# julienperriercornet/turbosqueeze

Hardware: AMD Instinct MI355X
Metric: encode+decode GB/s on enwik9-shaped input (round trip of uncompressed bytes) (higher is better)
Workload: dtype u8

## Files before the change

turbosqueeze_amd/csrc/tsq_enc_stage.cuh:

```cuda
#pragma once
#ifndef TSQ_LATE_FIX
#define TSQ_LATE_FIX 1
#endif
#ifndef TSQ_LM
#define TSQ_LM 4
#endif
#ifndef TSQ_LF
#define TSQ_LF 3
#endif
#ifndef TSQ_LM_LEAN
#define TSQ_LM_LEAN 4
#endif
#ifndef TSQ_LF_LEAN
#define TSQ_LF_LEAN 3
#endif

#include "tsq_common.cuh"
#include "tsq_experiment.h"
#include "tsq_enc_util.cuh"
#include "tsq_enc_builder.cuh"

namespace tsq {

typedef uint32_t u32x4_t __attribute__((ext_vector_type(4)));
// ... 222 lines not shown
    }
    return twin_in;
}

template <bool WINDOW>
__device__ __forceinline__ void stage_in(uint32_t n, lds_u8_t* lds, uint32_t lane)
{
    using StageCfg = StageCfgT<WINDOW>;
    volatile lds_u32_t* recs = (volatile lds_u32_t*)(lds + StageCfg::off_rec);
    lds_u32_t* ctl = (lds_u32_t*)(lds + StageCfg::off_ctl);
    const uint32_t n_tiles = (n >> 6) + 3u;
    uint32_t hashed_seen = 0, slot = 0;
    const uint64_t below_me = below(lane);
#ifdef TSQ_STATS
    unsigned long long st_[32] = {0};
#endif
    TSQ_BEGIN();
    for (uint32_t t = 0; t < n_tiles; ++t, slot = slot + 1u == StageCfg::R ? 0u : slot + 1u) {
        if (!stage_wait_seen(ctl, kCtlHashed, t + 1u, hashed_seen, 0)) break;
        volatile lds_u32_t* arr = recs + slot * StageCfg::REC_WORDS + StageCfg::ARR + lane * 4u;
        const u32x4_t gb = lds_ld4(arr + kGB);
        const uint32_t h = gb.y, own = gb.x;
        const uint64_t twin_in = in_tile_twins(h, own, below_me);
        lds_st2(arr + kGB + 2u, (uint32_t)twin_in, (uint32_t)(twin_in >> 32));
        TSQ_DELAY(10);
        stage_publish(ctl, kCtlIn, t + 1u, lane);
    }
#ifdef TSQ_STATS
    if (blockIdx.x == 0 && lane == 0) { g_enc_stats[34] = st_[22]; g_enc_stats[57] = st_[0]; g_enc_stats[58] = TSQ_TOTAL(); }
#endif
}

template <bool WINDOW>
__device__ __forceinline__ void stage_twins(uint32_t n, lds_u8_t* lds, uint32_t lane)
{
    using StageCfg = StageCfgT<WINDOW>;
    constexpr uint32_t LM = StageCfg::LM;
    volatile lds_u32_t* recs = (volatile lds_u32_t*)(lds + StageCfg::off_rec);
    lds_u32_t* ctl = (lds_u32_t*)(lds + StageCfg::off_ctl);
    const uint32_t n_tiles = (n >> 6) + 3u;
    uint32_t h_m1 = 0xFFFFFFFFu, h_m2 = 0xFFFFFFFFu, h_m3 = 0xFFFFFFFFu, h_m4 = 0xFFFFFFFFu;
    uint32_t hashed_seen = 0, slot = 0;
#ifdef TSQ_STATS
    unsigned long long st_[32] = {0};
#endif
    TSQ_BEGIN();
    for (uint32_t t = 0; t < n_tiles; ++t, slot = slot + 1u == StageCfg::R ? 0u : slot + 1u) {
        if (!stage_wait_seen(ctl, StageCfg::SPLIT_IN ? kCtlIn : kCtlHashed, t + 1u, hashed_seen, 0)) break;
        volatile lds_u32_t* rec = recs + slot * StageCfg::REC_WORDS;
        volatile lds_u32_t* arr = rec + StageCfg::ARR + lane * 4u;
        const u32x4_t gb = lds_ld4(arr + kGB);
        const uint32_t h = gb.y, own = gb.x;
        const uint32_t before = own & 0xFFu;
        if (!StageCfg::SPLIT_IN) {
            const uint64_t twin_in = in_tile_twins(h, own, below(lane));
            lds_st2(arr + kGB + 2u, (uint32_t)twin_in, (uint32_t)(twin_in >> 32));
        }
        uint64_t twin_p1 = 0, twin_p2 = 0, twin_p3 = 0, twin_p4 = 0;
        bool unsure = false;
        const uint32_t d0 = (t - (before >> 6)) & 3u;
        const uint32_t d = d0 ? d0 : 4u;
        const bool live = d <= t && d <= LM;
        if (__ballot(live) != 0ull) {
            const uint32_t q = before & 63u;
            const uint32_t dd = live ? d : 1u;
            const uint32_t qslot = slot >= dd ? slot - dd : slot + StageCfg::R - dd;
            volatile lds_u32_t* qa = recs + qslot * StageCfg::REC_WORDS + StageCfg::ARR + q * 4u;
            const u32x4_t qb = lds_ld4(qa + kGB);
            const u32x4_t qc = lds_ld4(qa + kGC);
            const uint32_t hq = qb.y;
            const uint64_t q_in = (uint64_t)qb.z | ((uint64_t)qb.w << 32);
            const uint64_t q_p1 = (uint64_t)qc.x | ((uint64_t)qc.y << 32);
            const uint64_t q_p2 = (uint64_t)qc.z | ((uint64_t)qc.w << 32);
            uint64_t q_p3 = 0;
            if (LM == 4u) { const u32x2_t qd = lds_ld2(qa + kGD); q_p3 = (uint64_t)qd.x | ((uint64_t)qd.y << 32); }
            const bool owns = live && StageCfg::fold(hq) == StageCfg::fold(h);
            const bool same = owns && hq == h;
            unsure = owns && hq != h;
            const uint64_t chain = q_in | (1ull << q);
            if (same) {
                twin_p1 = d == 1u ? chain : 0ull;
                twin_p2 = d == 2u ? chain : d == 1u ? q_p1 : 0ull;
                twin_p3 = d == 3u ? chain : d == 2u ? q_p1 : d == 1u ? q_p2 : 0ull;
                if (LM == 4u) twin_p4 = d == 4u ? chain : d == 3u ? q_p1 : d == 2u ? q_p2 : q_p3;
            }
        }
        {
            uint64_t maybe = __ballot(unsure);
            TSQ_CNT(20, __builtin_popcountll(maybe));
            while (maybe) {
                TSQ_CNT(21, 1);
                const uint32_t hl = rdlane(h, lsb64(maybe));
                const uint64_t g1 = __ballot(h_m1 == hl), g2 = __ballot(h_m2 == hl), g3 = __ballot(h_m3 == hl);
                const uint64_t g4 = LM == 4u ? __ballot(h_m4 == hl) : 0ull;
                const uint64_t grp_cur = __ballot(h == hl);
                if (h == hl) { twin_p1 = g1; twin_p2 = g2; twin_p3 = g3; twin_p4 = g4; }
                maybe &= ~grp_cur;
            }
        }
        lds_st4(arr + kGC, (uint32_t)twin_p1, (uint32_t)(twin_p1 >> 32), (uint32_t)twin_p2, (uint32_t)(twin_p2 >> 32));
        lds_st4(arr + kGD, (uint32_t)twin_p3, (uint32_t)(twin_p3 >> 32), (uint32_t)twin_p4, (uint32_t)(twin_p4 >> 32));
        TSQ_TRACE(2, t);
        TSQ_DELAY(1);
        stage_publish(ctl, 2, t + 1u, lane);
        h_m4 = h_m3; h_m3 = h_m2; h_m2 = h_m1; h_m1 = h;
    }
#ifdef TSQ_STATS
    if (blockIdx.x == 0 && lane == 0) { g_enc_stats[48] = st_[0]; g_enc_stats[49] = TSQ_TOTAL(); g_enc_stats[32] = st_[20]; g_enc_stats[33] = st_[21]; }
#endif
}

template <bool EXT, bool WINDOW>
__device__ __forceinline__ void stage_near(uint32_t n, lds_u8_t* lds, uint32_t lane)
{
    using StageCfg = StageCfgT<WINDOW>;
    volatile lds_u32_t* recs = (volatile lds_u32_t*)(lds + StageCfg::off_rec);
    lds_u32_t* ctl = (lds_u32_t*)(lds + StageCfg::off_ctl);
    const uint32_t n_tiles = (n >> 6) + 3u;
    uint32_t scanned_seen = 0, slot = 0;
#ifdef TSQ_STATS
    unsigned long long st_[32] = {0};
#endif
    TSQ_BEGIN();
    for (uint32_t t = 0; t < n_tiles; ++t, slot = slot + 1u == StageCfg::R ? 0u : slot + 1u) {
        if (!stage_wait_seen(ctl, 2, t + 1u, scanned_seen, 0)) break;
        volatile lds_u32_t* rec = recs + slot * StageCfg::REC_WORDS;
        volatile lds_u32_t* arr = rec + StageCfg::ARR + lane * 4u;
        const u32x2_t gi = lds_ld2(arr + kGB + 2u);
        const u32x4_t gc = lds_ld4(arr + kGC);
        u32x2_t gd; gd.x = 0; gd.y = 0;
        if (StageCfg::LM == 4u) gd = lds_ld2(arr + kGD);
        const uint32_t tin_lo = gi.x, tin_hi = gi.y, tp1_lo = gc.x, tp1_hi = gc.y, tp2_lo = gc.z, tp2_hi = gc.w, tp3_lo = gd.x, tp3_hi = gd.y;
        const bool in0 = (tin_lo | tin_hi) != 0u, in1 = (tp1_lo | tp1_hi) != 0u, in2 = (tp2_lo | tp2_hi) != 0u, in3 = (tp3_lo | tp3_hi) != 0u;
        uint32_t word = 0;
        if (__ballot(in0 || in1 || in2 || in3) != 0ull) {
            const uint32_t m_lo = in0 ? tin_lo : in1 ? tp1_lo : in2 ? tp2_lo : tp3_lo, m_hi = in0 ? tin_hi : in1 ? tp1_hi : in2 ? tp2_hi : tp3_hi;
            const uint32_t q = m_hi ? 63u - (uint32_t)__builtin_clz(m_hi) : 31u - (uint32_t)__builtin_clz(m_lo | 1u);
            const uint32_t back = in0 ? 0u : in1 ? 1u : in2 ? 2u : 3u;
            const uint32_t qslot = slot >= back ? slot - back : slot + StageCfg::R - back;
            const u32x4_t a = *(volatile lds_u32x4_t*)(rec + StageCfg::W16 + lane * 4u);
            const u32x4_t b = *(volatile lds_u32x4_t*)(recs + qslot * StageCfg::REC_WORDS + StageCfg::W16 + q * 4u);
            const uint32_t k = prefix16(make_uint4(a.x, a.y, a.z, a.w), make_uint4(b.x, b.y, b.z, b.w));
            if ((in0 || in1 || in2 || in3) && !(EXT && k >= 16u)) word = 0x8000u | (back << 12) | (q << 6) | k;
        }
        arr[kGB] = word;
        TSQ_DELAY(2);
        stage_publish(ctl, kCtlNear, t + 1u, lane);
    }
#ifdef TSQ_STATS
    if (blockIdx.x == 0 && lane == 0) { g_enc_stats[55] = st_[0]; g_enc_stats[56] = TSQ_TOTAL(); }
#endif
}

template <bool EXT, bool WINDOW>
__device__ __forceinline__ void stage_match(const uint8_t* src, uint64_t avail, uint32_t n, uint16_t* table, lds_u8_t* lds, uint32_t lane, uint32_t parity)
{
    using StageCfg = StageCfgT<WINDOW>;
    volatile lds_u32_t* recs = (volatile lds_u32_t*)(lds + StageCfg::off_rec);
    lds_u32_t* ctl = (lds_u32_t*)(lds + StageCfg::off_ctl);
    constexpr uint32_t kDMin = EXT ? 128u : 64u;
    constexpr uint32_t LM = StageCfg::LM;
    const uint32_t tail_from = n >= 5u ? n - 5u : 0u;
    const uint32_t n_tiles = (n >> 6) + 3u;
    uint32_t wbase = parity << 6;
    uint32_t scanned_seen = 0, committed_seen = 0;
#ifdef TSQ_STATS
    unsigned long long st_[32] = {0};
#endif
    TSQ_BEGIN();
    for (uint32_t t = parity; t < n_tiles; t += 2u) {
        MREG_BEGIN(10);
        if (!stage_wait_seen(ctl, 2, t + 1u, scanned_seen, 2)) break;
        TSQ_TRACE(3, t);
        volatile lds_u32_t* rec = recs + (t % StageCfg::R) * StageCfg::REC_WORDS;
        volatile lds_u32_t* arr = rec + StageCfg::ARR + lane * 4u;
        const u32x4_t gb = lds_ld4(arr + kGB);
        const u32x4_t wv = *(volatile lds_u32x4_t*)(rec + StageCfg::W16 + lane * 4u);
        const u32x4_t gc = lds_ld4(arr + kGC);
        const u32x4_t gd = lds_ld4(arr + kGD);
        const uint32_t h = gb.y;
        const uint4 w16 = make_uint4(wv.x, wv.y, wv.z, wv.w);
        const uint64_t twin_in = (uint64_t)gb.z | ((uint64_t)gb.w << 32);
        const uint64_t twin_p1 = (uint64_t)gc.x | ((uint64_t)gc.y << 32);
        const uint32_t tpw_any = LM == 4u ? (gc.z | gc.w | gd.x | gd.y) : (gc.z | gc.w);
        const uint32_t tpm_lo = LM == 4u ? gd.z : gd.x, tpm_hi = LM == 4u ? gd.w : gd.y;
        MREG_END(10);
        MREG_BEGIN(12);
#ifndef TSQ_X_NOCOMMITWAIT
        if (t >= LM + 1u && !stage_wait_seen(ctl, kCtlCommitted, t - LM, committed_seen, 3)) break;
#endif
        TSQ_TRACE(10, t);
#ifdef TSQ_X_FAKE_TABLE
        const uint32_t tv_old = table[h & 0xFFu];
#else
        const uint32_t tv_old = table[h];
#endif
        MREG_END(12);
        MREG_BEGIN(11);
        uint32_t tv = tv_old;
#ifdef TSQ_X_NOPATCH
        if (false) {
#else
        if (t >= LM) {
#endif
            volatile lds_u32_t* vis = recs + ((t - LM) % StageCfg::R) * StageCfg::REC_WORDS + 2u;
            uint32_t vis_lo, vis_hi;
            {
                const uint32_t seen_v = ((volatile lds_u32_t*)ctl)[5];
                uint32_t a = vis[0], b = vis[1];
                asm volatile("" ::: "memory");
                if (uniform(seen_v) < t - LM + 1u) {
                    if (!stage_wait_tight(ctl, 5, t - LM + 1u, 3)) break;
                    a = vis[0]; b = vis[1];
                }
                vis_lo = uniform(a); vis_hi = uniform(b);
            }
            TSQ_TRACE(4, t);
            const uint32_t hit_lo = tpm_lo & vis_lo, hit_hi = tpm_hi & vis_hi;
            const uint32_t q = hit_hi ? 63u - (uint32_t)__builtin_clz(hit_hi) : 31u - (uint32_t)__builtin_clz(hit_lo | 1u);
            if ((hit_lo | hit_hi) != 0u) tv = (((t - LM) << 6) + q) & 0xFFFFu;
        }
        MREG_END(11);
        const uint32_t p = (t << 6) + lane;
        const uint32_t cand0 = candidate_of(tv, p);
        MREG_BEGIN(13);
        uint4 cb;
        if (WINDOW) {
            int32_t wi = (int32_t)(wbase + lane) - (int32_t)(p - cand0);
            wi += wi < 0 ? (int32_t)StageCfg::WIN : 0;
            volatile lds_u32_t* wp = (volatile lds_u32_t*)(lds + StageCfg::off_win + ((uint32_t)wi & ~3u));
            const uint32_t d0 = wp[0], d1 = wp[1], d2 = wp[2], d3 = wp[3], d4 = wp[4];
            const uint32_t sh = (uint32_t)wi & 3u;
            cb = make_uint4(__builtin_amdgcn_alignbyte(d1, d0, sh), __builtin_amdgcn_alignbyte(d2, d1, sh),
                            __builtin_amdgcn_alignbyte(d3, d2, sh), __builtin_amdgcn_alignbyte(d4, d3, sh));
            if (cand0 + 19u > ((t + 1u) << 6) || p - cand0 > 65536u) cb = ld128z(src, cand0, avail);
        }
#ifdef TSQ_X_FAKE_CAND
        else cb = ld128z(src, p, avail);
#else
        else cb = ld128z(src, cand0, avail);
#endif
        uint32_t k0 = prefix16(w16, cb);
        MREG_END(13);
        MREG_BEGIN(14);
        if (EXT) {
            uint32_t more = 16;
            if (__ballot(k0 == more) != 0ull) {
                const uint32_t scanned = uniform(__hip_atomic_load(&ctl[2], __ATOMIC_RELAXED, __HIP_MEMORY_SCOPE_WORKGROUP));
                const bool in_window = WINDOW && scanned >= t + 2u;
                auto win16 = [&](int32_t wi) -> uint4 {
                    wi += wi < 0 ? (int32_t)StageCfg::WIN : 0;
                    wi -= wi >= (int32_t)StageCfg::WIN ? (int32_t)StageCfg::WIN : 0;
                    volatile lds_u32_t* wp = (volatile lds_u32_t*)(lds + StageCfg::off_win + ((uint32_t)wi & ~3u));
                    const uint32_t d0 = wp[0], d1 = wp[1], d2 = wp[2], d3 = wp[3], d4 = wp[4];
                    const uint32_t sh = (uint32_t)wi & 3u;
                    return make_uint4(__builtin_amdgcn_alignbyte(d1, d0, sh), __builtin_amdgcn_alignbyte(d2, d1, sh),
                                      __builtin_amdgcn_alignbyte(d3, d2, sh), __builtin_amdgcn_alignbyte(d4, d3, sh));
                };
                while (__ballot(k0 == more) != 0ull && more < 64u) {
                    TSQ_CNT(20, in_window ? 1 : 0); TSQ_CNT(21, 1);
                    if (k0 == more) {
                        if (in_window && p - cand0 <= 65536u)
                            k0 += prefix16(win16((int32_t)(wbase + lane + more)), win16((int32_t)(wbase + lane + more) - (int32_t)(p - cand0)));
                        else
                            k0 += prefix16(ld128z(src, (uint64_t)p + more, avail), ld128z(src, (uint64_t)cand0 + more, avail));
                    }
                    more += 16;
                }
            }
        }
        const uint32_t dist = p - cand0;
        const bool eq4 = k0 >= 4u;
        const bool far_enough = dist >= kDMin && dist <= 0xFFFEu;
        const bool tail = p >= tail_from;
        bool neart = false;
        if (__ballot((twin_in | twin_p1) != 0ull) != 0ull) {
            const uint64_t near_in = twin_in & ~below(lane >= 3u ? lane - 3u : 0u);
            const uint64_t near_prev = lane < 3u ? twin_p1 & ~below(61u + lane) : 0ull;
            neart = (near_in | near_prev) != 0ull && !tail;
        }
        const bool certain = eq4 && far_enough && !tail && !neart;
        const uint32_t nib = length_nibble(k0 < 4u ? 4u : k0);
        const uint32_t span_nat = certain ? nibble_span(nib) : 1u;
        const bool hard_l = (eq4 && !far_enough && dist >= 4u && !neart) || tail;
        const bool twin_l = (twin_in | twin_p1) != 0ull || tpw_any != 0u;
        lds_st2(arr + kGA, span_nat | (hard_l ? 0x100u : 0u) | (twin_l ? 0x200u : 0u) | (certain ? 0x400u : 0u) | (neart ? 0x800u : 0u) | (k0 << 16),
                cand0 | (nib << 24));
#ifdef TSQ_STATS
        if (t >= 3u) { st_[24] += (uint32_t)((uint32_t)__builtin_amdgcn_s_memtime() - uniform(ctl[40u + ((t - 3u) & 7u)])); st_[25] += 1; }
#endif
        TSQ_TRACE(5, t);
        TSQ_DELAY(3);
        stage_publish(ctl, parity ? kCtlMatchedOdd : 3u, t + 1u, lane);
        MREG_END(14);
        wbase = wbase + 128u >= StageCfg::WIN ? wbase + 128u - StageCfg::WIN : wbase + 128u;
    }
#ifdef TSQ_STATS
    if (blockIdx.x == 0 && lane == 0 && parity == 0u) { g_enc_stats[2] = st_[2]; g_enc_stats[3] = st_[3]; g_enc_stats[4] = TSQ_TOTAL(); g_enc_stats[13] = st_[13]; g_enc_stats[14] = st_[14]; g_enc_stats[35] = st_[20]; g_enc_stats[36] = st_[21]; g_enc_stats[51] = st_[24]; g_enc_stats[52] = st_[25]; }
#endif
}

template <bool WINDOW>
__device__ __forceinline__ void stage_commit(uint32_t n, uint16_t* table, lds_u8_t* lds, uint32_t lane)
{
    using StageCfg = StageCfgT<WINDOW>;
    volatile lds_u32_t* recs = (volatile lds_u32_t*)(lds + StageCfg::off_rec);
    lds_u32_t* ctl = (lds_u32_t*)(lds + StageCfg::off_ctl);
    const uint32_t n_tiles = (n >> 6) + 3u;
#ifdef TSQ_STATS
    unsigned long long st_[32] = {0};
#endif
    TSQ_BEGIN();
    for (uint32_t t = 0; t < n_tiles; ++t) {
        volatile lds_u32_t* rec = recs + (t % StageCfg::R) * StageCfg::REC_WORDS;
        volatile lds_u32_t* arr = rec + StageCfg::ARR + lane * 4u;
        if (!stage_wait(ctl, 5, t + 1u, 3)) break;
        TSQ_TRACE(12, t);
        const u32x4_t gb = lds_ld4(arr + kGB);
        const uint32_t h = gb.y, tin_lo = gb.z, tin_hi = gb.w;
        const uint64_t tw = __ballot((tin_lo | tin_hi) != 0u);
        lds_u32_t* visw = (lds_u32_t*)(rec + 2u);
        const uint64_t vis = (uint64_t)uniform(__hip_atomic_load(&visw[0], __ATOMIC_RELAXED, __HIP_MEMORY_SCOPE_WORKGROUP)) |
                             ((uint64_t)uniform(__hip_atomic_load(&visw[1], __ATOMIC_RELAXED, __HIP_MEMORY_SCOPE_WORKGROUP)) << 32);
        const uint32_t p = (t << 6) + lane;
#ifdef TSQ_X_FAKE_TABLE
#define TSQ_TBL(hh) ((hh) & 0xFFu)
#else
#define TSQ_TBL(hh) (hh)
#endif
        if (((vis & ~tw) >> lane) & 1ull) table[TSQ_TBL(h)] = (uint16_t)p;
        uint64_t late = vis & tw;
        while (late) {
            const uint32_t top = msb64(late);
            if (lane == top) table[TSQ_TBL(h)] = (uint16_t)p;
            late &= ~((uint64_t)rdlane(tin_lo, top) | ((uint64_t)rdlane(tin_hi, top) << 32) | (1ull << top));
        }
        asm volatile("s_waitcnt vmcnt(0)" ::: "memory");
        TSQ_TRACE(6, t);
        TSQ_DELAY(4);
        stage_publish(ctl, kCtlCommitted, t + 1u, lane);
    }
#ifdef TSQ_STATS
    if (blockIdx.x == 0 && lane == 0) { g_enc_stats[45] = st_[3] + st_[4]; g_enc_stats[46] = TSQ_TOTAL(); }
#endif
}

template <bool EXT, bool WINDOW>
__device__ __forceinline__ void stage_orbit(uint32_t n, lds_u8_t* lds, uint32_t lane, uint32_t parity)
{
    using StageCfg = StageCfgT<WINDOW>;
    volatile lds_u32_t* recs = (volatile lds_u32_t*)(lds + StageCfg::off_rec);
    lds_u32_t* ctl = (lds_u32_t*)(lds + StageCfg::off_ctl);
    constexpr uint32_t kDMin = EXT ? 128u : 64u;
    constexpr uint32_t LM = StageCfg::LM, LF = StageCfg::LF;
    const uint32_t tail_from = n >= 5u ? n - 5u : 0u;
    const uint32_t n_tiles = (n >> 6) + 3u;
#ifdef TSQ_STATS
    unsigned long long st_[32] = {0};
#endif
    TSQ_BEGIN();
    uint32_t scanned_seen = 0, parsed_seen = 0, near_seen = 0;
    for (uint32_t t = parity; t < n_tiles; t += 2u) {
        volatile lds_u32_t* rec = recs + (t % StageCfg::R) * StageCfg::REC_WORDS;
        volatile lds_u32_t* arr = rec + StageCfg::ARR + lane * 4u;
        uint32_t fix_sw = 0, fix_lw = 0;
        bool fix = false, clear_far = false;
        if (TSQ_LATE_FIX && t >= LF) {
            if (!stage_wait_seen(ctl, 2, t + 1u, scanned_seen, 6)) break;
            const u32x4_t gc = lds_ld4(arr + kGC);
            const u32x2_t gi = lds_ld2(arr + kGB + 2u);
            u32x2_t gd; gd.x = 0; gd.y = 0;
            if (LM == 4u) gd = lds_ld2(arr + kGD);
            const uint32_t tp_lo[4] = {0u, gc.x, gc.z, gd.x}, tp_hi[4] = {0u, gc.y, gc.w, gd.y};
            uint32_t nearer = gi.x | gi.y, far = 0;
#pragma unroll
            for (uint32_t k = 1; k < LM; ++k) { if (k < LF) nearer |= tp_lo[k] | tp_hi[k]; else far |= tp_lo[k] | tp_hi[k]; }
            const uint32_t p = (t << 6) + lane;
            const bool only_far = far != 0u && nearer == 0u && p < tail_from;
            if (__ballot(only_far) != 0ull) {
                if (!stage_wait_seen(ctl, 5, t - LF + 1u, parsed_seen, 5)) break;
                uint32_t hit_lo = 0, hit_hi = 0, back = 0;
#pragma unroll
                for (uint32_t k = LM - 1u; k >= LF; --k) {
                    lds_u32_t* vis = (lds_u32_t*)(recs + ((t - k) % StageCfg::R) * StageCfg::REC_WORDS + 2u);
                    const uint32_t v_lo = uniform(__hip_atomic_load(&vis[0], __ATOMIC_RELAXED, __HIP_MEMORY_SCOPE_WORKGROUP));
                    const uint32_t v_hi = uniform(__hip_atomic_load(&vis[1], __ATOMIC_RELAXED, __HIP_MEMORY_SCOPE_WORKGROUP));
                    const uint32_t h_lo = tp_lo[k] & v_lo, h_hi = tp_hi[k] & v_hi;
                    if ((h_lo | h_hi) != 0u) { hit_lo = h_lo; hit_hi = h_hi; back = k; }
                }
                clear_far = only_far;
                if (only_far && (hit_lo | hit_hi) != 0u) {
                    const uint32_t q = hit_hi ? 63u - (uint32_t)__builtin_clz(hit_hi) : 31u - (uint32_t)__builtin_clz(hit_lo);
                    const uint32_t cand = (t << 6) - (back << 6) + q;
                    const uint32_t tq = t - back;
                    const u32x4_t a = *(volatile lds_u32x4_t*)(rec + StageCfg::W16 + lane * 4u);
                    const u32x4_t b = *(volatile lds_u32x4_t*)(recs + (tq % StageCfg::R) * StageCfg::REC_WORDS + StageCfg::W16 + q * 4u);
                    const uint32_t k = prefix16(make_uint4(a.x, a.y, a.z, a.w), make_uint4(b.x, b.y, b.z, b.w));
                    if (p - cand >= kDMin && !(EXT && k >= 16u)) {
                        const bool eq4 = k >= 4u;
                        const uint32_t nib = length_nibble(eq4 ? k : 4u);
                        fix_sw = (eq4 ? nibble_span(nib) | 0x400u : 1u) | (k << 16);
                        fix_lw = cand | (nib << 24);
                        fix = true;
                    } else clear_far = false;
                }
            }
        }
        uint32_t sw, lw;
        {
            const uint32_t seen_v = ((volatile lds_u32_t*)ctl)[parity ? kCtlMatchedOdd : 3u];
            u32x2_t ga = lds_ld2(arr + kGA);
            asm volatile("" ::: "memory");
            if (uniform(seen_v) < t + 1u) {
                if (!stage_wait_tight(ctl, parity ? kCtlMatchedOdd : 3u, t + 1u, 6)) break;
                ga = lds_ld2(arr + kGA);
            }
            sw = ga.x; lw = ga.y;
        }
        TSQ_TRACE(11, t);
        if (clear_far) fix_sw |= 0x1000u;
        if (fix) { sw = fix_sw; lw = fix_lw; }
        else if (clear_far) sw |= 0x1000u;
        const uint32_t self = lane | ((sw & 0x100u) ? 0x80u : 0u);
        const uint32_t c = lane + (sw & 0xFFu);
        const uint32_t there = (uint32_t)__builtin_amdgcn_ds_bpermute((int)((c & 63u) << 2), (int)self);
        uint32_t nx = c >= 64u ? (c | 0x80u) : there;
        uint64_t orb = 1ull << lane;
#pragma unroll
        for (int round = 0; round < 6; ++round) {
            const int at = (int)((nx & 63u) << 2);
            const uint32_t nx2 = (uint32_t)__builtin_amdgcn_ds_bpermute(at, (int)nx);
            const uint32_t olo = (uint32_t)__builtin_amdgcn_ds_bpermute(at, (int)(uint32_t)orb);
            const uint32_t ohi = (uint32_t)__builtin_amdgcn_ds_bpermute(at, (int)(uint32_t)(orb >> 32));
            if ((nx & 0x80u) == 0u) { nx = nx2; orb |= (uint64_t)olo | ((uint64_t)ohi << 32); }
        }
        if (!stage_wait_seen(ctl, kCtlNear, t + 1u, near_seen, 6)) break;
        const bool hard_l = (sw & 0x100u) != 0u;
        const uint32_t orb_lo = hard_l ? 0u : (uint32_t)orb, orb_hi = hard_l ? 0u : (uint32_t)(orb >> 32);
        const uint32_t halt = hard_l ? lane : (nx & 0x7Fu);
        lds_st4(arr + kGA, sw | (halt << 24), lw, orb_lo, orb_hi);
#ifdef TSQ_STATS
        if (t >= 3u) { st_[24] += (uint32_t)((uint32_t)__builtin_amdgcn_s_memtime() - uniform(ctl[40u + ((t - 3u) & 7u)])); st_[25] += 1; }
#endif
        TSQ_TRACE(7, t);
        TSQ_DELAY(5);
        stage_publish(ctl, parity ? kCtlOrbitOdd : kCtlOrbitEven, t + 1u, lane);
    }
#ifdef TSQ_STATS
    if (blockIdx.x == 0 && lane == 0 && parity == 0u) { g_enc_stats[6] = st_[6] + st_[5]; g_enc_stats[7] = TSQ_TOTAL(); g_enc_stats[53] = st_[24]; g_enc_stats[54] = st_[25]; }
#endif
}

#if defined(TSQ_FUSED_OFF)
template <bool EXT, bool WINDOW> struct FusedMO { static constexpr bool value = false; };
#elif defined(TSQ_FUSED_ALL)
template <bool EXT, bool WINDOW> struct FusedMO { static constexpr bool value = true; };
#else
template <bool EXT, bool WINDOW> struct FusedMO { static constexpr bool value = EXT || !WINDOW; };
#endif
template <bool EXT, bool WINDOW>
__device__ __forceinline__ uint32_t orbit_word(uint32_t t)
{ return FusedMO<EXT, WINDOW>::value ? kCtlOrbitQ + (t & 3u) : ((t & 1u) ? kCtlOrbitOdd : kCtlOrbitEven); }
template <bool EXT, bool WINDOW>
__device__ __forceinline__ uint32_t orbit_word_after(uint32_t t)
{ return FusedMO<EXT, WINDOW>::value ? kCtlOrbitQ + ((t + 1u) & 3u) : ((t & 1u) ? kCtlOrbitEven : kCtlOrbitOdd); }

template <bool EXT, bool WINDOW>
__device__ __forceinline__ void stage_match_orbit(const uint8_t* src, uint64_t avail, uint32_t n, uint16_t* table, lds_u8_t* lds, uint32_t lane, uint32_t which)
{
    using StageCfg = StageCfgT<WINDOW>;
    volatile lds_u32_t* recs = (volatile lds_u32_t*)(lds + StageCfg::off_rec);
    lds_u32_t* ctl = (lds_u32_t*)(lds + StageCfg::off_ctl);
    constexpr uint32_t kDMin = EXT ? 128u : 64u;
    constexpr uint32_t LM = StageCfg::LM, LF = StageCfg::LF;
    const uint32_t tail_from = n >= 5u ? n - 5u : 0u;
    const uint32_t n_tiles = (n >> 6) + 3u;
    uint32_t wbase = which << 6;
    uint32_t scanned_seen = 0, committed_seen = 0, parsed_seen = 0, near_seen = 0;
#ifdef TSQ_STATS
    unsigned long long st_[32] = {0};
#endif
    TSQ_BEGIN();
    for (uint32_t t = which; t < n_tiles; t += 4u) {
        if (!stage_wait_seen(ctl, 2, t + 1u, scanned_seen, 2)) break;
        TSQ_TRACE(3, t);
        volatile lds_u32_t* rec = recs + (t % StageCfg::R) * StageCfg::REC_WORDS;
        volatile lds_u32_t* arr = rec + StageCfg::ARR + lane * 4u;
        const u32x4_t gb = lds_ld4(arr + kGB);
        const u32x4_t wv = *(volatile lds_u32x4_t*)(rec + StageCfg::W16 + lane * 4u);
        const u32x4_t gc = lds_ld4(arr + kGC);
        const u32x4_t gd = lds_ld4(arr + kGD);
        const uint32_t h = gb.y;
        const uint4 w16 = make_uint4(wv.x, wv.y, wv.z, wv.w);
        const uint64_t twin_in = (uint64_t)gb.z | ((uint64_t)gb.w << 32);
        const uint64_t twin_p1 = (uint64_t)gc.x | ((uint64_t)gc.y << 32);
        const uint32_t tpw_any = LM == 4u ? (gc.z | gc.w | gd.x | gd.y) : (gc.z | gc.w);
        const uint32_t tpm_lo = LM == 4u ? gd.z : gd.x, tpm_hi = LM == 4u ? gd.w : gd.y;
        if (t >= LM + 1u && !stage_wait_seen(ctl, kCtlCommitted, t - LM, committed_seen, 3)) break;
        TSQ_TRACE(10, t);
        const uint32_t tv_old = table[h];
        uint32_t tv = tv_old;
        if (t >= LM) {
            volatile lds_u32_t* vis = recs + ((t - LM) % StageCfg::R) * StageCfg::REC_WORDS + 2u;
            uint32_t vis_lo, vis_hi;
            {
                const uint32_t seen_v = ((volatile lds_u32_t*)ctl)[5];
                uint32_t a = vis[0], b = vis[1];
                asm volatile("" ::: "memory");
                if (uniform(seen_v) < t - LM + 1u) {
                    if (!stage_wait_tight(ctl, 5, t - LM + 1u, 3)) break;
                    a = vis[0]; b = vis[1];
                }
                vis_lo = uniform(a); vis_hi = uniform(b);
            }
            TSQ_TRACE(4, t);
            const uint32_t hit_lo = tpm_lo & vis_lo, hit_hi = tpm_hi & vis_hi;
            const uint32_t q = hit_hi ? 63u - (uint32_t)__builtin_clz(hit_hi) : 31u - (uint32_t)__builtin_clz(hit_lo | 1u);
            if ((hit_lo | hit_hi) != 0u) tv = (((t - LM) << 6) + q) & 0xFFFFu;
        }
        uint32_t fix_sw = 0, fix_lw = 0;
        bool fix = false, clear_far = false;
        const uint32_t p = (t << 6) + lane;
        auto late_fix = [&]() -> bool {
        if (TSQ_LATE_FIX && t >= LF) {
            const uint32_t tp_lo[4] = {0u, gc.x, gc.z, gd.x}, tp_hi[4] = {0u, gc.y, gc.w, gd.y};
            uint32_t nearer = gb.z | gb.w, far = 0;
#pragma unroll
            for (uint32_t k = 1; k < LM; ++k) { if (k < LF) nearer |= tp_lo[k] | tp_hi[k]; else far |= tp_lo[k] | tp_hi[k]; }
            const bool only_far = far != 0u && nearer == 0u && p < tail_from;
            if (__ballot(only_far) != 0ull) {
                if (!stage_wait_seen(ctl, 5, t - LF + 1u, parsed_seen, 5)) return false;
                uint32_t hit_lo = 0, hit_hi = 0, back = 0;
#pragma unroll
                for (uint32_t k = LM - 1u; k >= LF; --k) {
                    lds_u32_t* vis = (lds_u32_t*)(recs + ((t - k) % StageCfg::R) * StageCfg::REC_WORDS + 2u);
                    const uint32_t v_lo = uniform(__hip_atomic_load(&vis[0], __ATOMIC_RELAXED, __HIP_MEMORY_SCOPE_WORKGROUP));
                    const uint32_t v_hi = uniform(__hip_atomic_load(&vis[1], __ATOMIC_RELAXED, __HIP_MEMORY_SCOPE_WORKGROUP));
                    const uint32_t h_lo = tp_lo[k] & v_lo, h_hi = tp_hi[k] & v_hi;
                    if ((h_lo | h_hi) != 0u) { hit_lo = h_lo; hit_hi = h_hi; back = k; }
                }
                clear_far = only_far;
                if (only_far && (hit_lo | hit_hi) != 0u) {
                    const uint32_t q = hit_hi ? 63u - (uint32_t)__builtin_clz(hit_hi) : 31u - (uint32_t)__builtin_clz(hit_lo);
                    const uint32_t cand = (t << 6) - (back << 6) + q;
                    const uint32_t tq = t - back;
                    const u32x4_t b = *(volatile lds_u32x4_t*)(recs + (tq % StageCfg::R) * StageCfg::REC_WORDS + StageCfg::W16 + q * 4u);
                    const uint32_t k = prefix16(w16, make_uint4(b.x, b.y, b.z, b.w));
                    if (p - cand >= kDMin && !(EXT && k >= 16u)) {
                        const bool eq4f = k >= 4u;
                        const uint32_t nibf = length_nibble(eq4f ? k : 4u);
                        fix_sw = (eq4f ? nibble_span(nibf) | 0x400u : 1u) | (k << 16);
                        fix_lw = cand | (nibf << 24);
                        fix = true;
                    } else clear_far = false;
                }
            }
        }
        return true;
        };
        const uint32_t cand0 = candidate_of(tv, p);
        uint4 cb;
        if (WINDOW) {
            int32_t wi = (int32_t)(wbase + lane) - (int32_t)(p - cand0);
            wi += wi < 0 ? (int32_t)StageCfg::WIN : 0;
            volatile lds_u32_t* wp = (volatile lds_u32_t*)(lds + StageCfg::off_win + ((uint32_t)wi & ~3u));
            const uint32_t d0 = wp[0], d1 = wp[1], d2 = wp[2], d3 = wp[3], d4 = wp[4];
            const uint32_t sh = (uint32_t)wi & 3u;
            cb = make_uint4(__builtin_amdgcn_alignbyte(d1, d0, sh), __builtin_amdgcn_alignbyte(d2, d1, sh),
                            __builtin_amdgcn_alignbyte(d3, d2, sh), __builtin_amdgcn_alignbyte(d4, d3, sh));
            if (cand0 + 19u > ((t + 1u) << 6) || p - cand0 > 65536u) cb = ld128z(src, cand0, avail);
        }
        else cb = ld128z(src, cand0, avail);
        uint32_t k0 = prefix16(w16, cb);
        if (EXT) {
            uint32_t more = 16;
            if (__ballot(k0 == more) != 0ull) {
                const uint32_t scanned = uniform(__hip_atomic_load(&ctl[2], __ATOMIC_RELAXED, __HIP_MEMORY_SCOPE_WORKGROUP));
                const bool in_window = WINDOW && scanned >= t + 2u;
                auto win16 = [&](int32_t wi) -> uint4 {
                    wi += wi < 0 ? (int32_t)StageCfg::WIN : 0;
                    wi -= wi >= (int32_t)StageCfg::WIN ? (int32_t)StageCfg::WIN : 0;
                    volatile lds_u32_t* wp = (volatile lds_u32_t*)(lds + StageCfg::off_win + ((uint32_t)wi & ~3u));
                    const uint32_t d0 = wp[0], d1 = wp[1], d2 = wp[2], d3 = wp[3], d4 = wp[4];
                    const uint32_t sh = (uint32_t)wi & 3u;
                    return make_uint4(__builtin_amdgcn_alignbyte(d1, d0, sh), __builtin_amdgcn_alignbyte(d2, d1, sh),
                                      __builtin_amdgcn_alignbyte(d3, d2, sh), __builtin_amdgcn_alignbyte(d4, d3, sh));
                };
                while (__ballot(k0 == more) != 0ull && more < 64u) {
                    if (k0 == more) {
                        if (in_window && p - cand0 <= 65536u)
                            k0 += prefix16(win16((int32_t)(wbase + lane + more)), win16((int32_t)(wbase + lane + more) - (int32_t)(p - cand0)));
                        else
                            k0 += prefix16(ld128z(src, (uint64_t)p + more, avail), ld128z(src, (uint64_t)cand0 + more, avail));
                    }
                    more += 16;
                }
            }
        }
        const uint32_t dist = p - cand0;
        const bool eq4 = k0 >= 4u;
        const bool far_enough = dist >= kDMin && dist <= 0xFFFEu;
        const bool tail = p >= tail_from;
        bool neart = false;
        if (__ballot((twin_in | twin_p1) != 0ull) != 0ull) {
            const uint64_t near_in = twin_in & ~below(lane >= 3u ? lane - 3u : 0u);
            const uint64_t near_prev = lane < 3u ? twin_p1 & ~below(61u + lane) : 0ull;
            neart = (near_in | near_prev) != 0ull && !tail;
        }
        const bool certain = eq4 && far_enough && !tail && !neart;
        const uint32_t nib = length_nibble(k0 < 4u ? 4u : k0);
        const uint32_t span_nat = certain ? nibble_span(nib) : 1u;
        const bool hard_m = (eq4 && !far_enough && dist >= 4u && !neart) || tail;
        const bool twin_l = (twin_in | twin_p1) != 0ull || tpw_any != 0u;
        uint32_t sw = span_nat | (hard_m ? 0x100u : 0u) | (twin_l ? 0x200u : 0u) | (certain ? 0x400u : 0u) | (neart ? 0x800u : 0u) | (k0 << 16);
        uint32_t lw = cand0 | (nib << 24);
        TSQ_TRACE(5, t);
        TSQ_TRACE(11, t);
        if (!late_fix()) break;
        if (fix) { sw = fix_sw; lw = fix_lw; }
        if (clear_far) sw |= 0x1000u;
        const uint32_t self = lane | ((sw & 0x100u) ? 0x80u : 0u);
        const uint32_t c = lane + (sw & 0xFFu);
        const uint32_t there = (uint32_t)__builtin_amdgcn_ds_bpermute((int)((c & 63u) << 2), (int)self);
        uint32_t nx = c >= 64u ? (c | 0x80u) : there;
        uint64_t orb = 1ull << lane;
#pragma unroll
        for (int round = 0; round < 6; ++round) {
            const int at = (int)((nx & 63u) << 2);
            const uint32_t nx2 = (uint32_t)__builtin_amdgcn_ds_bpermute(at, (int)nx);
            const uint32_t olo = (uint32_t)__builtin_amdgcn_ds_bpermute(at, (int)(uint32_t)orb);
            const uint32_t ohi = (uint32_t)__builtin_amdgcn_ds_bpermute(at, (int)(uint32_t)(orb >> 32));
            if ((nx & 0x80u) == 0u) { nx = nx2; orb |= (uint64_t)olo | ((uint64_t)ohi << 32); }
        }
        if (!stage_wait_seen(ctl, kCtlNear, t + 1u, near_seen, 6)) break;
        const bool hard_l = (sw & 0x100u) != 0u;
        const uint32_t orb_lo = hard_l ? 0u : (uint32_t)orb, orb_hi = hard_l ? 0u : (uint32_t)(orb >> 32);
        const uint32_t halt = hard_l ? lane : (nx & 0x7Fu);
        lds_st4(arr + kGA, sw | (halt << 24), lw, orb_lo, orb_hi);
        TSQ_TRACE(7, t);
        TSQ_DELAY(5);
        stage_publish(ctl, kCtlOrbitQ + (t & 3u), t + 1u, lane);
        wbase = wbase + 256u >= StageCfg::WIN ? wbase + 256u - StageCfg::WIN : wbase + 256u;
    }
#ifdef TSQ_STATS
    if (blockIdx.x == 0 && lane == 0 && which == 0u) { g_enc_stats[2] = st_[2]; g_enc_stats[3] = st_[3]; g_enc_stats[4] = TSQ_TOTAL(); g_enc_stats[6] = st_[6] + st_[5]; g_enc_stats[7] = TSQ_TOTAL(); }
#endif
}

__device__ __forceinline__ uint32_t s_sel(uint32_t c, uint32_t a, uint32_t b)
{ uint32_t d; asm("s_cmp_lg_u32 %1, 0\n\ts_cselect_b32 %0, %2, %3" : "=s"(d) : "s"(c), "s"(a), "s"(b) : "scc"); return d; }
__device__ __forceinline__ uint64_t s_sel64(uint32_t c, uint64_t a, uint64_t b)
{ uint64_t d; asm("s_cmp_lg_u32 %1, 0\n\ts_cselect_b64 %0, %2, %3" : "=s"(d) : "s"(c), "s"(a), "s"(b) : "scc"); return d; }
__device__ __forceinline__ void s_sel_64_32(uint32_t c, uint64_t a1, uint64_t b1, uint32_t a2, uint32_t b2, uint64_t& d1, uint32_t& d2)
{ asm("s_cmp_lg_u32 %2, 0\n\ts_cselect_b64 %0, %3, %4\n\ts_cselect_b32 %1, %5, %6" : "=&s"(d1), "=&s"(d2) : "s"(c), "s"(a1), "s"(b1), "s"(a2), "s"(b2) : "scc"); }
__device__ __forceinline__ void s_selnz64_64_32(uint64_t x, uint64_t a1, uint64_t b1, uint32_t a2, uint32_t b2, uint64_t& d1, uint32_t& d2)
{ asm("s_cmp_lg_u64 %2, 0\n\ts_cselect_b64 %0, %3, %4\n\ts_cselect_b32 %1, %5, %6" : "=&s"(d1), "=&s"(d2) : "s"(x), "s"(a1), "s"(b1), "s"(a2), "s"(b2) : "scc"); }
__device__ __forceinline__ uint32_t s_selnz64(uint64_t x, uint32_t a, uint32_t b)
{ uint32_t d; asm("s_cmp_lg_u64 %1, 0\n\ts_cselect_b32 %0, %2, %3" : "=s"(d) : "s"(x), "s"(a), "s"(b) : "scc"); return d; }
__device__ __forceinline__ uint32_t s_nz64(uint64_t x)
{ uint32_t d; asm("s_cmp_lg_u64 %1, 0\n\ts_cselect_b32 %0, 1, 0" : "=s"(d) : "s"(x) : "scc"); return d; }
__device__ __forceinline__ uint32_t s_nz(uint32_t x)
{ uint32_t d; asm("s_min_u32 %0, %1, 1" : "=s"(d) : "s"(x) : "scc"); return d; }
__device__ __forceinline__ uint32_t s_lt(uint32_t a, uint32_t b)
{ uint32_t d; asm("s_cmp_lt_u32 %1, %2\n\ts_cselect_b32 %0, 1, 0" : "=s"(d) : "s"(a), "s"(b) : "scc"); return d; }
__device__ __forceinline__ uint32_t s_ge(uint32_t a, uint32_t b)
{ uint32_t d; asm("s_cmp_ge_u32 %1, %2\n\ts_cselect_b32 %0, 1, 0" : "=s"(d) : "s"(a), "s"(b) : "scc"); return d; }
__device__ __forceinline__ uint32_t s_ne(uint32_t a, uint32_t b)
{ uint32_t d; asm("s_cmp_lg_u32 %1, %2\n\ts_cselect_b32 %0, 1, 0" : "=s"(d) : "s"(a), "s"(b) : "scc"); return d; }
__device__ __forceinline__ uint32_t s_eq(uint32_t a, uint32_t b)
{ uint32_t d; asm("s_cmp_eq_u32 %1, %2\n\ts_cselect_b32 %0, 1, 0" : "=s"(d) : "s"(a), "s"(b) : "scc"); return d; }
__device__ __forceinline__ uint32_t s_offset_ok(uint32_t offset)
{ uint32_t d; asm("s_add_u32 %0, %1, -4\n\ts_cmp_lt_u32 %0, 0xfffb\n\ts_cselect_b32 %0, 1, 0" : "=&s"(d) : "s"(offset) : "scc"); return d; }
__device__ __forceinline__ uint32_t s_msb64(uint64_t x)
{ uint32_t d; asm("s_flbit_i32_b64 %0, %1\n\ts_xor_b32 %0, %0, 63" : "=s"(d) : "s"(x) : "scc"); return d; }
__device__ __forceinline__ uint32_t s_lsb64(uint64_t x)
{ uint32_t d; asm("s_ff1_i32_b64 %0, %1" : "=s"(d) : "s"(x)); return d; }


template <bool EXT, bool WINDOW>
__device__ __forceinline__ void stage_walk(const uint8_t* src, uint64_t avail, uint32_t n, lds_u8_t* lds, uint32_t lane)
{
    using StageCfg = StageCfgT<WINDOW>;
    volatile lds_u32_t* evq = (volatile lds_u32_t*)(lds + StageCfg::off_evq);
    volatile lds_u32_t* recs = (volatile lds_u32_t*)(lds + StageCfg::off_rec);
    lds_u32_t* ctl = (lds_u32_t*)(lds + StageCfg::off_ctl);
    const uint32_t tail_from = uniform(n >= 5u ? n - 5u : 0u);
    constexpr uint32_t LM = StageCfg::LM, LF = StageCfg::LF;

    uint32_t ev_head = 0, ev_tail_seen = 0, n_query = 0;
    uint32_t v = 1, done = 0;
    uint32_t last_m = 0;
    uint64_t vall_p1 = 0, vall_p2 = 0, vall_p3 = 0;
#ifdef TSQ_STATS
    unsigned long long st_[32] = {0};
#endif

    auto ev_wait_space = [&]() {
#ifdef TSQ_STATS
        const unsigned long long w0_ = __builtin_amdgcn_s_memtime();
#endif
        while (ev_head - ev_tail_seen >= StageCfg::EQ) {
            ev_tail_seen = uniform(__hip_atomic_load(&ctl[kCtlEvTail], __ATOMIC_RELAXED, __HIP_MEMORY_SCOPE_WORKGROUP));
            if (ev_head - ev_tail_seen >= StageCfg::EQ) { TSQ_SPIN_AT(ctl, 46u); __builtin_amdgcn_s_sleep(1); }
        }
#ifdef TSQ_STATS
        st_[9] += __builtin_amdgcn_s_memtime() - w0_;
#endif
    };
    auto ev_push = [&](uint32_t kind, uint32_t a, uint32_t b, uint32_t c) {
        if (ev_head - ev_tail_seen >= StageCfg::EQ) ev_wait_space();
        volatile lds_u32_t* e = evq + (ev_head % StageCfg::EQ) * StageCfg::EV_WORDS;
        uint32_t hv = kind;
        asm volatile("v_writelane_b32 %0, %1, 1" : "+v"(hv) : "s"(a));
        asm volatile("v_writelane_b32 %0, %1, 2" : "+v"(hv) : "s"(b));
        asm volatile("v_writelane_b32 %0, %1, 3" : "+v"(hv) : "s"(c));
        if (lane < 4u) e[lane] = hv;
        TSQ_JIT(ev_head * 64u + 40u);
        TSQ_LDS_RELEASE();
        ev_head++;
        __hip_atomic_store(&ctl[kCtlEvHead], ev_head, __ATOMIC_RELAXED, __HIP_MEMORY_SCOPE_WORKGROUP);
    };
    auto words_at = [&](uint32_t slot, uint32_t pos) -> uint4 {
        const u32x4_t q = *(volatile lds_u32x4_t*)(recs + slot * StageCfg::REC_WORDS + StageCfg::W16 + (pos & 63u) * 4u);
        return make_uint4(q.x, q.y, q.z, q.w);
    };

    uint32_t wbase = 0;
    uint32_t rec_slot = 0;
    uint32_t spanword, lane_word, nx, orb_lo, orb_hi, tin_lo, tin_hi, tp1_lo, tp1_hi, tp2r_lo, tp2r_hi, tp3r_lo = 0, tp3r_hi = 0, nearw, seen_v;
    auto load_record = [&](volatile lds_u32_t* arr) {
        const u32x4_t ga = lds_ld4(arr + kGA), gb = lds_ld4(arr + kGB), gc = lds_ld4(arr + kGC);
        spanword = ga.x; lane_word = ga.y; orb_lo = ga.z; orb_hi = ga.w;
        nearw = gb.x; tin_lo = gb.z; tin_hi = gb.w;
        tp1_lo = gc.x; tp1_hi = gc.y; tp2r_lo = gc.z; tp2r_hi = gc.w;
        if (LM == 4u) { const u32x2_t gd = lds_ld2(arr + kGD); tp3r_lo = gd.x; tp3r_hi = gd.y; }
        nx = spanword >> 24;
    };
    seen_v = ((volatile lds_u32_t*)ctl)[orbit_word<EXT, WINDOW>(0u)];
    load_record(recs + StageCfg::ARR + lane * 4u);
    asm volatile("" ::: "memory");
    TSQ_BEGIN();
    for (uint32_t t = 0; done == 0u; ++t, wbase = wbase + 64u == StageCfg::WIN ? 0u : wbase + 64u, rec_slot = rec_slot + 1u == StageCfg::R ? 0u : rec_slot + 1u) {
        const uint32_t base = t << 6;
        uint64_t vall = 0;
        {
            REG_BEGIN(0); REG_END(0);
            REG_BEGIN(1);
            const uint32_t orbit_at = orbit_word<EXT, WINDOW>(t);
            volatile lds_u32_t* arr = recs + rec_slot * StageCfg::REC_WORDS + StageCfg::ARR + lane * 4u;
            if (uniform(seen_v) < t + 1u) {
#ifdef TSQ_STATS
                const unsigned long long w0_ = __builtin_amdgcn_s_memtime();
#endif
                while (!stage_ready(ctl, orbit_at, t + 1u)) { TSQ_SPIN(ctl); }
#ifdef TSQ_STATS
                st_[8] += __builtin_amdgcn_s_memtime() - w0_;
#endif
                load_record(arr);
            }
            TSQ_CNT(15, 1);
            TSQ_TRACE(8, t);
            const uint32_t settled = (spanword & 0x1000u) ? 0u : 0xFFFFFFFFu;
            const uint32_t tp2_lo = LF <= 2u ? tp2r_lo & settled : tp2r_lo, tp2_hi = LF <= 2u ? tp2r_hi & settled : tp2r_hi;
            const uint32_t tp3_lo = tp3r_lo & settled, tp3_hi = tp3r_hi & settled;
            uint64_t handed = 0;
            const uint64_t near_m = __ballot((spanword & 0x800u) != 0u);
            const uint64_t certain_m = __ballot((spanword & 0x400u) != 0u);
            uint32_t prev_hit = (tp1_lo & (uint32_t)vall_p1) | (tp1_hi & (uint32_t)(vall_p1 >> 32)) |
                                (tp2_lo & (uint32_t)vall_p2) | (tp2_hi & (uint32_t)(vall_p2 >> 32));
            if (LM == 4u) prev_hit |= (tp3_lo & (uint32_t)vall_p3) | (tp3_hi & (uint32_t)(vall_p3 >> 32));
            const uint32_t k0 = (spanword >> 16) & 0xFFu;
            const uint32_t cand0 = lane_word & 0xFFFFFFu;

            uint32_t L = v - base;
            auto segment = [&]() {
                REG_BEGIN(2);
                const uint32_t L0 = L;
                const uint32_t o_lo = rdlane(orb_lo, L0), o_hi = rdlane(orb_hi, L0);
                uint64_t V = (uint64_t)o_lo | ((uint64_t)o_hi << 32);
                L = rdlane(nx, L0);
                const uint64_t seen = vall | V;
                const uint32_t in_lo = tin_lo & (uint32_t)seen, in_hi = tin_hi & (uint32_t)(seen >> 32);
#ifdef TSQ_X_NOHAZ
                uint64_t bad = 0;
#else
                uint64_t bad = __ballot((in_lo | in_hi | prev_hit) != 0u) & V;
#endif
                if (__builtin_expect((V & near_m) != 0ull, 0)) {
                    uint32_t a_lo = in_lo, a_hi = in_hi, b_lo = tp1_lo, b_hi = tp1_hi;
                    asm volatile("; near twins" : "+v"(a_lo), "+v"(a_hi), "+v"(b_lo), "+v"(b_hi));
                    const uint32_t pv_lo = b_lo & (uint32_t)vall_p1, pv_hi = b_hi & (uint32_t)(vall_p1 >> 32);
                    const bool has_in = (a_lo | a_hi) != 0u, has_prev = (pv_lo | pv_hi) != 0u;
                    const uint32_t nearest = a_hi ? 63u - (uint32_t)__builtin_clz(a_hi) : 31u - (uint32_t)__builtin_clz(a_lo | 1u);
// ... 753 lines not shown
```

Baseline: 22.75.

## Prefetch next tile's hash-table lookup early in orbit match stage

```diff
diff --git a/turbosqueeze_amd/csrc/tsq_enc_stage.cuh b/turbosqueeze_amd/csrc/tsq_enc_stage.cuh
--- a/turbosqueeze_amd/csrc/tsq_enc_stage.cuh
+++ b/turbosqueeze_amd/csrc/tsq_enc_stage.cuh
@@ -398,6 +398,22 @@
 #endif
 }
 
+#ifdef TSQ_X_FAKE_TABLE
+#define TSQ_TBL(hh) ((hh) & 0xFFu)
+#else
+#define TSQ_TBL(hh) (hh)
+#endif
+#define TSQ_EARLY_GATHER(fresh)                                                                                                       \
+    do {                                                                                                                              \
+        if (EARLY && h_known && !have_next) {                                                                                         \
+            if ((fresh) && committed_seen < need_next) {                                                                              \
+                committed_seen = uniform(__hip_atomic_load(&ctl[kCtlCommitted], __ATOMIC_RELAXED, __HIP_MEMORY_SCOPE_WORKGROUP));     \
+                asm volatile("" ::: "memory");                                                                                        \
+            }                                                                                                                         \
+            if (committed_seen >= need_next) { tv_next = table[TSQ_TBL(h_next)]; have_next = true; }                                  \
+        }                                                                                                                             \
+    } while (0)
+
 template <bool EXT, bool WINDOW>
 __device__ __forceinline__ void stage_match(const uint8_t* src, uint64_t avail, uint32_t n, uint16_t* table, lds_u8_t* lds, uint32_t lane, uint32_t parity)
 {
@@ -436,11 +452,7 @@
         if (t >= LM + 1u && !stage_wait_seen(ctl, kCtlCommitted, t - LM, committed_seen, 3)) break;
 #endif
         TSQ_TRACE(10, t);
-#ifdef TSQ_X_FAKE_TABLE
-        const uint32_t tv_old = table[h & 0xFFu];
-#else
-        const uint32_t tv_old = table[h];
-#endif
+        const uint32_t tv_old = table[TSQ_TBL(h)];
         MREG_END(12);
         MREG_BEGIN(11);
         uint32_t tv = tv_old;
@@ -569,11 +581,6 @@
         const uint64_t vis = (uint64_t)uniform(__hip_atomic_load(&visw[0], __ATOMIC_RELAXED, __HIP_MEMORY_SCOPE_WORKGROUP)) |
                              ((uint64_t)uniform(__hip_atomic_load(&visw[1], __ATOMIC_RELAXED, __HIP_MEMORY_SCOPE_WORKGROUP)) << 32);
         const uint32_t p = (t << 6) + lane;
-#ifdef TSQ_X_FAKE_TABLE
-#define TSQ_TBL(hh) ((hh) & 0xFFu)
-#else
-#define TSQ_TBL(hh) (hh)
-#endif
         if (((vis & ~tw) >> lane) & 1ull) table[TSQ_TBL(h)] = (uint16_t)p;
         uint64_t late = vis & tw;
         while (late) {
@@ -723,6 +730,9 @@
     const uint32_t n_tiles = (n >> 6) + 3u;
     uint32_t wbase = which << 6;
     uint32_t scanned_seen = 0, committed_seen = 0, parsed_seen = 0, near_seen = 0;
+    constexpr bool EARLY = !WINDOW && !EXT;
+    uint32_t h_next = 0, tv_next = 0;
+    bool have_next = false;
 #ifdef TSQ_STATS
     unsigned long long st_[32] = {0};
 #endif
@@ -742,9 +752,20 @@
         const uint64_t twin_p1 = (uint64_t)gc.x | ((uint64_t)gc.y << 32);
         const uint32_t tpw_any = LM == 4u ? (gc.z | gc.w | gd.x | gd.y) : (gc.z | gc.w);
         const uint32_t tpm_lo = LM == 4u ? gd.z : gd.x, tpm_hi = LM == 4u ? gd.w : gd.y;
-        if (t >= LM + 1u && !stage_wait_seen(ctl, kCtlCommitted, t - LM, committed_seen, 3)) break;
-        TSQ_TRACE(10, t);
-        const uint32_t tv_old = table[h];
+        uint32_t tv_old = tv_next;
+        if (!have_next) {
+            if (t >= LM + 1u && !stage_wait_seen(ctl, kCtlCommitted, t - LM, committed_seen, 3)) break;
+            TSQ_TRACE(10, t);
+            tv_old = table[TSQ_TBL(h)];
+        }
+        const uint32_t t_next = t + 4u, need_next = t_next >= LM + 1u ? t_next - LM : 0u;
+        uint32_t sc_next = 0, cm_next = 0;
+        if (EARLY) {
+            sc_next = ((volatile lds_u32_t*)ctl)[2];
+            h_next = recs[(t_next % StageCfg::R) * StageCfg::REC_WORDS + StageCfg::ARR + lane * 4u + kGB + 1u];
+            cm_next = ((volatile lds_u32_t*)ctl)[kCtlCommitted];
+            asm volatile("" ::: "memory");
+        }
         uint32_t tv = tv_old;
         if (t >= LM) {
             volatile lds_u32_t* vis = recs + ((t - LM) % StageCfg::R) * StageCfg::REC_WORDS + 2u;
@@ -764,6 +785,10 @@
             const uint32_t q = hit_hi ? 63u - (uint32_t)__builtin_clz(hit_hi) : 31u - (uint32_t)__builtin_clz(hit_lo | 1u);
             if ((hit_lo | hit_hi) != 0u) tv = (((t - LM) << 6) + q) & 0xFFFFu;
         }
+        if (EARLY) { scanned_seen = uniform(sc_next); committed_seen = uniform(cm_next); }
+        const bool h_known = EARLY && scanned_seen >= t_next + 1u;
+        have_next = false;
+        TSQ_EARLY_GATHER(false);
         uint32_t fix_sw = 0, fix_lw = 0;
         bool fix = false, clear_far = false;
         const uint32_t p = (t << 6) + lane;
@@ -818,6 +843,7 @@
         }
         else cb = ld128z(src, cand0, avail);
         uint32_t k0 = prefix16(w16, cb);
+        TSQ_EARLY_GATHER(true);
         if (EXT) {
             uint32_t more = 16;
             if (__ballot(k0 == more) != 0ull) {
@@ -885,6 +911,7 @@
         lds_st4(arr + kGA, sw | (halt << 24), lw, orb_lo, orb_hi);
         TSQ_TRACE(7, t);
         TSQ_DELAY(5);
+        TSQ_EARLY_GATHER(true);
         stage_publish(ctl, kCtlOrbitQ + (t & 3u), t + 1u, lane);
         wbase = wbase + 256u >= StageCfg::WIN ? wbase + 256u - StageCfg::WIN : wbase + 256u;
     }
```

Result: no change. 22.79, median of 4 (+0.1%).
